# astooke/accel_rl

Hardware: AMD Instinct MI355X
Metric: env-steps/sec (whole node), 256-env PPO Atari (higher is better)
Workload: dtype f32; 1 GPU; PPO breakout, 256 envs/GPU, horizon 5, spec-1 CNN (fp32), minibatch 512/GPU x 4 epochs, adam; synthetic fixed-frame emulator; hipGraph rollout; total_envs=256, global_minibatch=512, parallelism=single

## Files before the change

accel_rl_amd/_lib.py:

```python
import ctypes as C
import os

import torch

_PKG = os.path.dirname(os.path.abspath(__file__))
LIB_PATH = os.path.join(_PKG, "libaccel_rl_hip.so")

ARL_ABI_VERSION = 4
PROMO_NEP50, PROMO_LEGACY, PROMO_ASSOC = 0, 1, 2
PPO_TIE_THEANO, PPO_TIE_MATH, PPO_TIE_BOTH = 0, 1, 2
OPT_ADAM, OPT_RMSPROP = 0, 1
MAX_ACTIONS = 18
REPLAY_MAX_HORIZON = 16
RAW_H, RAW_W, OBS_H, OBS_W = 210, 160, 104, 80
OPT_PARTIALS = 1024

_vp, _i32, _i64, _f32, _f64 = C.c_void_p, C.c_int32, C.c_int64, C.c_float, C.c_double


class ArlGame(C.Structure):
    _fields_ = [("bank", _vp), ("n_frames", _i32), ("n_actions", _i32),
                ("action_set", _i32 * MAX_ACTIONS), ("start_lives", _i32),
                ("life_period", _i32), ("frame_skip", _i32), ("n_stack", _i32),
                ("clip_reward", _i32), ("episodic_lives", _i32), ("resample_mode", _i32)]
# ... 157 lines not shown
    "arl_is_weights": (_i32, [_vp, _i64, _f64, _vp, _vp]),
    "arl_priority_diffs": (_i32, [_vp, _vp, _i64, _f64, _vp, _vp]),
    "arl_catdqn_act": (_i32, [_vp, _vp, _vp, _i64, _i32, _i32, _i32, _i32, _vp, _vp, _vp]),
    "arl_catdqn_loss": (_i32, [_vp] * 8 + [_i64, _i32, _i32, _i32, _i32, _f32, _f32, _f32, _vp, _vp, _vp, _vp]),
    "arl_catdqn_loss_parts": (_i32, [_vp] * 8 + [_i64, _i32, _i32, _i32, _i32, _f32, _f32, _f32, _vp, _vp, _vp, _vp, _i32,
                               _vp]),
    "arl_dqn_act": (_i32, [_vp, _vp, _i64, _i32, _i32, _i32, _vp, _vp, _vp]),
    "arl_dqn_loss": (_i32, [_vp] * 7 + [_i64, _i32, _i32, _i32, _f32, _f32, _vp, _vp, _vp, _vp]),
    "arl_lstm_cell_fwd": (_i32, [_vp, _i64, _vp, _vp, _i64, _i64, _i32, _vp, _i64, _vp, _i64, _vp, _i64, _vp]),
    "arl_lstm_cell_bwd": (_i32, [_vp, _i64, _vp, _vp, _vp, _i64, _vp, _i64, _vp, _i64, _i64, _i32, _vp, _i64, _vp, _vp]),
    "arl_gru_cell_fwd": (_i32, [_vp, _i64, _vp, _vp, _i64, _i64, _i32, _vp, _i64, _vp, _i64, _vp]),
    "arl_gru_cell_bwd": (_i32, [_vp, _i64, _vp, _vp, _vp, _i64, _vp, _i64, _i64, _i32, _vp, _i64, _vp, _i64, _vp, _vp]),
    "arl_rnn_cell_fwd": (_i32, [_vp, _i64, _vp, _i64, _i32, _vp, _i64, _vp]),
    "arl_rnn_cell_bwd": (_i32, [_vp, _i64, _vp, _vp, _i64, _i64, _i32, _vp, _i64, _vp]),
    "arl_opt_step": (_i32, [C.POINTER(ArlOptState), _i32, _f32, _f32, _f32, _f32, _f32, _f32, _vp]),
    "arl_opt_step_noclip": (_i32, [C.POINTER(ArlOptState), _i32, _f32, _f32, _f32, _f32, _f32, _i32, _vp, _vp, _vp]),
    "arl_opt_finish": (_i32, [C.POINTER(ArlOptState), _i32, _f32, _vp, _vp, _vp]),
    "arl_opt_step_noclip_split": (_i32, [C.POINTER(ArlOptState), _i32, _f32, _f32, _f32, _f32, _f32, _i32, _vp, _vp,
                                         _i64, _i64, _i32, _vp]),
    "arl_opt_finish_split": (_i32, [C.POINTER(ArlOptState), _i32, _f32, _vp, _vp, _i64, _vp]),
    "arl_corun_job_init": (_i32, [C.POINTER(ArlCorunJob), C.POINTER(ArlOptState), _i32, _f32, _f32, _f32, _f32, _f32,
                                  _i32, _vp, _vp, _i64, _i64]),
    "arl_corun_job_run": (_i32, [C.POINTER(ArlCorunJob), _vp]),
    "arl_noisy_normals": (_i32, [_i64, _i64, _i32, _i32, _i64, _i32, _i32, _vp, _vp, _vp, _vp]),
    "arl_noisy_noise": (_i32, [_vp, C.POINTER(ArlNoisyLayer), _i32, _i64, _i32, _vp]),
    "arl_noisy_dense_combine": (_i32, [C.POINTER(ArlFoldItem), _vp, C.POINTER(ArlFoldItem), _vp, _vp, _i64, _i32, _i32,
                                       _vp, _vp, _vp, _vp, _vp]),
    "arl_noisy_dense_bwd_prep": (_i32, [_vp, _vp, _i64, _i32, _vp, _vp, _vp, _vp]),
    "arl_noisy_dense_bwd_dx": (_i32, [_vp, _vp, _vp, _i64, _i32, _vp, _vp]),
    "arl_noisy_draws": (_i32, [_vp, C.POINTER(ArlNoisyDraw), _i32, _i64, _i32, _vp]),
    "arl_noisy_duel_combine": (_i32, [C.POINTER(ArlFoldItem), _vp, C.POINTER(ArlFoldItem), C.POINTER(ArlFoldItem), _vp,
                                      _vp, _i64, _i32, _i32, _i32, _vp, _vp, _vp, _vp, _vp]),
    "arl_noisy_duel_bwd_prep": (_i32, [_vp, _vp, _i64, _i32, _i32, _vp, _vp, _vp, _vp, _vp]),
    "arl_noisy_duel_bwd_dx": (_i32, [_vp, _vp, _vp, _vp, _vp, _i64, _i32, _vp, _vp]),
    "arl_noisy_catdqn_loss_limits": (_i32, [C.POINTER(_i32), C.POINTER(_i32), C.POINTER(_i32)]),
    "arl_noisy_catdqn_loss_parts": (_i32, [C.POINTER(ArlNoisyLogitSrc), C.POINTER(ArlNoisyLogitSrc),
                                           C.POINTER(ArlNoisyLogitSrc), _vp, _vp, _vp, _vp, _vp, _i64, _i32, _i32, _i32,
                                           _i32, _f32, _f32, _f32, _vp, _vp, _vp, C.POINTER(ArlDgradWt), _i32, _vp]),
}

_DEV_SIGNATURES = {
    "arl_dev_conv_trace_buffer": (None, [_vp]),
    "arl_dev_conv_force_generic": (None, [_i32]),
    "arl_dev_conv_variant": (None, [_i32]),
    "arl_dev_fwd_tile": (None, [_i32]),
    "arl_dev_dgrad_wt": (None, [_i32]),
# ... 507 lines not shown
    def pg_head_loss(self, h, w_head, b_head, actions, advantages, returns, old_prob, valids, idx, lr_mult,
                     inv_count, n_actions, kind, clip_param, v_loss_coeff, ent_loss_coeff,
                     dout, dh, dw_head, db_head, loss4, workspace, stream=None, relu_mask_dh=False,
                 tie_rule=PPO_TIE_THEANO, dgrad_weights=None):
        batch, hid = h.shape
        assert self._n + 3 <= FOLD_MAX_ITEMS, "too many pending folds"
        first = C.byref(self._items[self._n])
        self._n += 3
        wt_items, n_wt = None, 0
        if dgrad_weights:
            n_wt = len(dgrad_weights)
            assert n_wt <= DGRAD_WT_MAX
            wt_items = (ArlDgradWt * n_wt)()
            for it, (w, wt, geom) in zip(wt_items, dgrad_weights):
                it.w, it.wt, it.geom = ptr(w), ptr(wt), C.pointer(geom)
        _check(load().arl_pg_head_loss_parts(
            ptr(h), w_head.data_ptr(), b_head.data_ptr(), ptr(actions), ptr(advantages), ptr(returns),
            ptr(old_prob), ptr(valids), ptr(idx), ptr(lr_mult), ptr(inv_count), batch, hid, n_actions,
            kind, int(tie_rule), float(clip_param), float(v_loss_coeff), float(ent_loss_coeff), int(bool(relu_mask_dh)), ptr(dout),
            ptr(dh), dw_head.data_ptr(), db_head.data_ptr(), ptr(loss4), ptr(workspace), first,
            None if wt_items is None else C.cast(wt_items, _vp), n_wt, stream_ptr(stream)),
            "arl_pg_head_loss_parts")

    def run(self, stream=None):
        n, self._n = self._n, 0
        _check(load().arl_fold_many(self._items, n, stream_ptr(stream)), "arl_fold_many")



def replay_append(rb, observations, actions, rewards, dones, horizon, idx, discount, promo=PROMO_NEP50,
                  stream=None):
    _want(observations, torch.uint8, "observations")
    _want(actions, torch.uint8, "actions")
    _want(rewards, torch.float32, "rewards")
    _check(load().arl_replay_append(C.byref(rb), ptr(observations), ptr(actions), ptr(rewards), ptr(dones),
                                    horizon, idx, float(discount), promo, stream_ptr(stream)), "arl_replay_append")


def replay_extract(rb, env_idxs, step_idxs, obs, next_obs, actions, returns, terminals, stream=None):
    _want(env_idxs, torch.int32, "env_idxs")
    _want(step_idxs, torch.int32, "step_idxs")
    _check(load().arl_replay_extract(C.byref(rb), ptr(env_idxs), ptr(step_idxs), env_idxs.numel(), ptr(obs),
                                     ptr(next_obs), ptr(actions), ptr(returns), ptr(terminals),
                                     stream_ptr(stream)), "arl_replay_extract")


def sumtree_find(tree, levels, uniforms, out, stream=None):
    _want(tree, torch.float64, "tree")
    _want(uniforms, torch.float64, "uniforms")
# ... 297 lines not shown
```

accel_rl_amd/csrc/arl_optim_dev.h:

```cpp
#pragma once

#include "arl_common.h"

namespace arl {

__device__ __forceinline__ double wave_sum_d(double x) {
#pragma unroll
    for (int off = 32; off > 0; off >>= 1) x += __shfl_down(x, off, 64);
    return x;
}

__device__ __forceinline__ double block_sum_d(double x, double* lds) {
    x = wave_sum_d(x);
    const int lane = threadIdx.x & 63, w = threadIdx.x >> 6, nw = blockDim.x >> 6;
    if (lane == 0) lds[w] = x;
    __syncthreads();
    if (threadIdx.x == 0) {
        double s = 0;
        for (int i = 0; i < nw; ++i) s += lds[i];
        lds[0] = s;
    }
    __syncthreads();
    const double r = lds[0];
    __syncthreads();
// ... 70 lines not shown
        if (METHOD == ARL_OPT_ADAM) st_nt(v4 + i, v);
    }
    const long long n = o.n_params;
    if (c.finish && block == 0 && threadIdx.x < (n & 3)) {
        const long long i = ((n >> 2) << 2) + threadIdx.x;
        const float g = o.grads[i];
        float p = o.params[i], m = o.slot0[i], v = (METHOD == ARL_OPT_ADAM) ? o.slot1[i] : 0.f;
        s += (double)g * g;
        update_one<METHOD>(p, g, m, v, c.avg, 1.f, lr, a_t, c.b1, c.b2, c.eps);
        o.params[i] = p;
        o.slot0[i] = m;
        if (METHOD == ARL_OPT_ADAM) o.slot1[i] = v;
    }
    s = block_sum_d(s, lds);
    if (threadIdx.x == 0) {
        c.norm_parts[(long long)c.k * ARL_OPT_NORM_BLOCKS + c.block0 + block] = s;
        if (c.finish && block == 0) { c.step_pp[(c.k + 1) & 1] = t; o.step_count[0] = t; }
    }
    if (block == 0)
        for (int i = nblocks + threadIdx.x; i < c.slots; i += blockDim.x)
            c.norm_parts[(long long)c.k * ARL_OPT_NORM_BLOCKS + c.block0 + i] = 0.0;
}

inline void opt_split_plan(long long n_params, long long hole_count, int* rest, int* hole) {
    const long long n4 = n_params >> 2, h4 = hole_count >> 2;
    *rest = (int)stream_grid(n4 - h4, 256);
    if (h4 > 0 && *rest > ARL_OPT_NORM_BLOCKS / 2) *rest = ARL_OPT_NORM_BLOCKS / 2;
    long long hb = (h4 + 511) / 512;
    if (hb > ARL_OPT_NORM_BLOCKS - *rest) hb = ARL_OPT_NORM_BLOCKS - *rest;
    *hole = h4 > 0 ? (int)(hb < 1 ? 1 : hb) : 0;
}

int make_opt_seg(OptSeg* c, const arl_opt_state* opt, int32_t method, float learning_rate, float avg_factor,
                 float beta1_or_rho, float beta2, float epsilon, int32_t k, float* step_pp, double* norm_parts,
                 int64_t hole_first, int64_t hole_count, int part, int* blocks);
int launch_opt_seg(const OptSeg& c, int blocks, hipStream_t s);

}
```

accel_rl_amd/csrc/mfma_conv.hip:

```cpp
#include "mfma_conv_impl.h"
#include "dgrad_wt_dev.h"

using namespace arlc;

namespace arlc {
thread_local CallCtx t_ctx = {9, nullptr, false};
unsigned long long* g_trace = nullptr;
bool g_force_generic = false;
int g_fwd_tile = -1;
}

namespace {
constexpr int FOLD_WIDE = 128, FOLD_THREADS = 1024;
int g_fold_wide = FOLD_WIDE;
bool g_dgrad_wt = true;

struct FoldSlot { int64_t i; int zg, zgn, row0, o; };
__device__ __forceinline__ FoldSlot fold_slot(int splits, int local_block, int wide_from) {
    FoldSlot f;
    const int tid = threadIdx.x;
    f.o = tid & 15;
    if (splits >= wide_from) { f.zg = tid >> 4; f.zgn = 64; f.row0 = 0; f.i = (int64_t)local_block * 16 + f.o; }
    else {
        const int grp = tid >> 8;
// ... 55 lines not shown
};

__global__ __launch_bounds__(FOLD_THREADS) void fold_many_kernel(const FoldManyArgs a) {
    __shared__ float4 lds[64][16];
    int it = 0;
    while (it + 1 < a.n && (int)blockIdx.x >= a.block_start[it + 1]) ++it;
    const float4* part = reinterpret_cast<const float4*>(a.items[it].part);
    float4* out = reinterpret_cast<float4*>(a.items[it].out);
    const int64_t total4 = a.items[it].total >> 2;
    const int splits = a.items[it].splits;
    const FoldSlot f = fold_slot(splits, (int)blockIdx.x - a.block_start[it], a.wide_from);
    const float4 s = fold_sum(part, splits, total4, f, lds);
    const int64_t i = f.i;
    if (f.zg == 0 && i < total4) {
        const int64_t valid = a.items[it].valid;
        if (valid <= 0 || 4 * i + 3 < valid) {
            out[i] = s;
        } else {
            float* o1 = reinterpret_cast<float*>(out + i);
            if (4 * i < valid) o1[0] = s.x;
            if (4 * i + 1 < valid) o1[1] = s.y;
            if (4 * i + 2 < valid) o1[2] = s.z;
        }
    }
}

int launch_fold(const float* part, int splits, int64_t total, const float* bias, int n_bias, int relu,
                float* out, hipStream_t s, const float* mask = nullptr) {
    const int64_t total4 = total >> 2;
    hipLaunchKernelGGL(fold_splits_kernel, dim3((unsigned)fold_blocks(splits, total4)), dim3(FOLD_THREADS), 0, s,
                       (const float4*)part, splits, total4, (const float4*)bias, n_bias >> 2, relu,
                       (const float4*)mask, (float4*)out, g_fold_wide);
    return arl::check_launch("fold_splits_kernel");
}

}

extern "C" int64_t arl_conv_workspace_bytes(void) { return (int64_t)64 << 20; }

extern "C" void arl_dev_conv_trace_buffer(void* device_u64_or_null) { g_trace = (unsigned long long*)device_u64_or_null; }

extern "C" void arl_dev_conv_force_generic(int32_t on) { g_force_generic = on != 0; }

extern "C" void arl_dev_fold_wide_from(int32_t splits) { g_fold_wide = splits > 0 ? splits : FOLD_WIDE; }

extern "C" void arl_dev_fwd_tile(int32_t v) { g_fwd_tile = ((v >= 0 && v <= 2) || v == 6 || v == 7) ? v : -1; }
// ... 557 lines not shown
        for (int ph = 0; ph < st; ++ph)
            for (int pw = 0; pw < st; ++pw) {
                q.i0[ph * st + pw] = (ph + g.pad_h) % st;
                q.j0[ph * st + pw] = (pw + g.pad_w) % st;
            }
        a.block_start[i] = blocks;
        blocks += (q.total + 255) / 256;
    }
    a.block_start[n] = blocks; a.n = n;
    *blocks_out = blocks;
    return 0;
}
}

extern "C" int arl_conv2d_dgrad_weights(const arl_dgrad_wt* items, int32_t n, void* stream) {
    arlw::DgradWtArgs a;
    int blocks = 0;
    int rc = arlw::dgrad_wt_plan(items, n, &a, &blocks);
    if (rc) return rc;
    hipLaunchKernelGGL(dgrad_weights_kernel, dim3((unsigned)blocks), dim3(256), 0, (hipStream_t)stream, a);
    return arl::check_launch("dgrad_weights_kernel");
}

extern "C" int arl_fold_many(const arl_fold_item* items, int32_t n, void* stream) {
    ARL_REQUIRE(items || n == 0, ARL_E_ARG, "null pointer");
    ARL_REQUIRE(n >= 0 && n <= ARL_FOLD_MAX_ITEMS, ARL_E_RANGE, "too many fold items");
    FoldManyArgs a = {};
    int blocks = 0;
    for (int i = 0; i < n; ++i) {
        if (items[i].splits <= 0) continue;
        ARL_REQUIRE(items[i].part && items[i].out && items[i].total > 0 && (items[i].total & 3) == 0, ARL_E_ARG,
                    "fold item: null pointer or length not a multiple of 4");
        ARL_REQUIRE(arl::aligned16(items[i].part) && arl::aligned16(items[i].out), ARL_E_ALIGN, "16-byte alignment");
        a.items[a.n] = items[i];
        a.block_start[a.n++] = blocks;
        blocks += fold_blocks(items[i].splits, items[i].total >> 2);
    }
    if (a.n == 0) return 0;
    a.block_start[a.n] = blocks;
    a.wide_from = g_fold_wide;
    hipLaunchKernelGGL(fold_many_kernel, dim3((unsigned)blocks), dim3(FOLD_THREADS), 0, (hipStream_t)stream, a);
    return arl::check_launch("fold_many_kernel");
}
```

accel_rl_amd/optimizers/base.py:

```python
import numpy as np
import torch

from accel_rl_amd import _lib

NORM_LOG_LEN = 64


def iterate_mb_idxs(batch_size, data_length, shuffle=False):
    if shuffle:
        order = np.arange(data_length)
        np.random.shuffle(order)
    for lo in range(0, data_length - batch_size + 1, batch_size):
        yield order[lo:lo + batch_size] if shuffle else np.arange(lo, lo + batch_size)


def iterate_traj_idxs(batch_size, data_length, horizon=1, shuffle=False):
    if data_length % horizon or batch_size % horizon or data_length % batch_size:
        raise AssertionError("batch_size and data_length must be multiples of horizon, data_length of batch_size")
    rows = np.arange(data_length).reshape(-1, horizon)
    order = np.arange(data_length // horizon)
    per = batch_size // horizon
    if shuffle:
        np.random.shuffle(order)
    for lo in range(0, len(order), per):
# ... 11 lines not shown

    @property
    def parallelism_tag(self):
        raise NotImplementedError

    def _setup_bucket(self, target, lr_mult, givens=None):
        self._target = target
        dev = target.device
        n = target.flat_params.numel()
        self._slot0 = torch.zeros(n, dtype=torch.float32, device=dev)
        self._slot1 = torch.zeros(n, dtype=torch.float32, device=dev) \
            if self._update_method.name == "adam" else None
        self._step_count = torch.zeros(1, dtype=torch.float32, device=dev)
        if not isinstance(lr_mult, torch.Tensor):
            lr_mult = torch.full((1,), float(lr_mult), dtype=torch.float32, device=dev)
        self._lr_mult = lr_mult
        self._partials = torch.zeros(_lib.OPT_PARTIALS, dtype=torch.float64, device=dev)
        self._norm_log = torch.zeros(NORM_LOG_LEN, dtype=torch.float32, device=dev)
        self._n_updates = 0
        self._step_pp = self._norm_parts = None
        self._hole = None
        self._call_hole = None
        self._hole_count = 0
        st = _lib.ArlOptState()
        st.n_params = n
        st.params, st.grads = target.flat_params.data_ptr(), target.flat_grads.data_ptr()
        st.slot0 = self._slot0.data_ptr()
        st.slot1 = self._slot1.data_ptr() if self._slot1 is not None else None
        st.step_count, st.lr_mult = self._step_count.data_ptr(), self._lr_mult.data_ptr()
        st.partials, st.grad_norm_log = self._partials.data_ptr(), self._norm_log.data_ptr()
        st.norm_log_len = NORM_LOG_LEN
        self._opt_state = st
        a = self._update_args
        if self._update_method.name == "adam":
            self._kernel_args = (a["beta1"], a["beta2"], a["epsilon"])
        else:
            self._kernel_args = (a["rho"], 0.0, a["epsilon"])

    def _backward(self, losses, minibatch):
        return losses(minibatch)[3]

    def _apply_update(self, avg_factor=1.0):
        b1, b2, eps = self._kernel_args
        if self._grad_norm_clip is None:
            self._noclip_state()
            k = self._n_updates % self._opt_state.norm_log_len
            hole, self._hole = self._hole, None
            if k == 0:
                self._call_hole = hole
                self._hole_count = hole[1] if hole else 0
            elif self._hole_count and hole is None:
                hole = self._call_hole
                _lib.corun_job_run(_lib.corun_job(self._opt_state, self._update_method.kernel_id, self._learning_rate,
                                                  avg_factor, b1, b2, eps, k, self._step_pp, self._norm_parts,
                                                  hole[0], hole[1]))
            if self._hole_count:
                hole = self._call_hole
                _lib.opt_step_noclip_split(self._opt_state, self._update_method.kernel_id, self._learning_rate,
                                           avg_factor, b1, b2, eps, k, self._step_pp, self._norm_parts, hole[0],
                                           hole[1], 0)
            else:
                _lib.opt_step_noclip(self._opt_state, self._update_method.kernel_id, self._learning_rate, avg_factor,
                                     b1, b2, eps, k, self._step_pp, self._norm_parts)
            self._pending_avg = avg_factor
        else:
            _lib.opt_step(self._opt_state, self._update_method.kernel_id, self._learning_rate,
                          avg_factor, self._grad_norm_clip, b1, b2, eps)
        self._n_updates += 1

    corun_update = True

    def _noclip_state(self):
        if self._step_pp is None:
            dev = self._target.device
            self._step_pp = self._step_count.repeat(2).contiguous()
            self._norm_parts = torch.zeros(_lib.OPT_NORM_SLOTS * _lib.OPT_NORM_BLOCKS, dtype=torch.float64, device=dev)
        elif self._n_updates % self._opt_state.norm_log_len == 0 and not self._hole:
            self._step_pp.copy_(self._step_count.expand(2))

    def _corun_hook(self, avg_factor=1.0):
        if self._grad_norm_clip is not None or not self.corun_update:
            return None
        b1, b2, eps = self._kernel_args

        def hook(first, count):
            self._noclip_state()
            k = self._n_updates % self._opt_state.norm_log_len
            if k and (self._hole_count == 0 or self._call_hole != (first, count)):
                return None
            self._hole = (first, count)
            return _lib.corun_job(self._opt_state, self._update_method.kernel_id, self._learning_rate, avg_factor,
                                  b1, b2, eps, k, self._step_pp, self._norm_parts, first, count)
        return hook

    def _set_updates_per_call(self, count):
        count = max(1, min(int(count), NORM_LOG_LEN))
        if self._opt_state.norm_log_len != count:
            assert self._n_updates % count == 0 or self._n_updates == 0
            self._opt_state.norm_log_len = count

    def _recent_grad_norms(self, count):
        assert 0 < count <= self._opt_state.norm_log_len
        self._finish_updates(count)
        out = self._norm_log[:count]
        return out if (out.is_cuda and torch.cuda.is_current_stream_capturing()) else out.clone()

    def _finish_updates(self, count):
        if self._grad_norm_clip is None and self._step_pp is not None:
            _lib.opt_finish(self._opt_state, count, self._pending_avg, self._step_pp, self._norm_parts,
                            hole_count=self._hole_count)
```

accel_rl_amd/optimizers/single.py:

```python
import numpy as np
import torch

from accel_rl_amd import _lib

from accel_rl_amd.optimizers.base import BaseOptimizer, iterate_mb_idxs


class A2cOptimizer(BaseOptimizer):

    def __init__(self, learning_rate, update_method, update_method_args=None, grad_norm_clip=None):
        self._learning_rate = learning_rate
        self._update_method = update_method
        self._update_args = update_method.resolve(**(update_method_args or dict()))
        self._grad_norm_clip = grad_norm_clip

    def initialize(self, inputs, losses, constraints, target, givens=None, lr_mult=1):
        self._input_names = list(inputs)
        self._losses = losses
        self._setup_bucket(target, lr_mult, givens)

    def optimize(self, inputs):
        self.prepare_host(len(inputs[0]))
        return self.device_updates(inputs)

# ... 43 lines not shown

    def prepare_host(self, data_length):
        bs = self._minibatch_size
        flat = [mb for _ in range(self._epochs)
                for mb in iterate_mb_idxs(bs, data_length, self._shuffle)]
        if self._idx_host is None:
            shape = (max(len(flat), 1), bs)
            self._idx_host = torch.zeros(shape, dtype=torch.int32).pin_memory()
            self._idx_dev = torch.zeros(shape, dtype=torch.int32, device=self._target.device)
        self._n_minibatches = len(flat)
        self._set_updates_per_call(len(flat))
        if flat:
            self._idx_host.copy_(torch.from_numpy(np.stack(flat).astype(np.int32)))

    def device_updates(self, inputs):
        data = dict(zip(self._input_names, inputs))
        if not self._n_minibatches:
            return [], []
        _lib.copy_bytes(self._idx_dev, self._idx_host)
        if self._overlap_allreduce:
            return self._overlapped_minibatches(data)
        losses = []
        corun = self._corun_hook() if self.parallelism_tag == "single" else None
        try:
            for k in range(self._n_minibatches):
                mb = self._minibatch(data, self._idx_dev[k])
                if corun is not None:
                    mb["dense_w_hook"] = corun
                losses.append(self._backward(self._losses, mb))
                self._share_grad()
                self._apply_update(self._avg_factor())
        finally:
            self._hole = None
        return losses, self._recent_grad_norms(self._n_minibatches)

    def _minibatch(self, data, idx):
        return dict(data, idx=idx)

    _overlap_allreduce = False

    def _overlapped_minibatches(self, data):
        losses = []
        for k in range(self._n_minibatches):
            pending = []
            mb = self._minibatch(data, self._idx_dev[k])
            mb["split_hook"] = lambda: pending.append(self._share_grad_async(tail=True))
            losses.append(self._backward(self._losses, mb))
            pending.append(self._share_grad_async(tail=False) if pending else self._share_grad_async(None))
            self._wait_all(pending)
            self._apply_update(self._avg_factor())
        return losses, self._recent_grad_norms(self._n_minibatches)

    @staticmethod
    def _wait_all(pending):
        for work in pending:
            if work is not None:
# ... 15 lines not shown
```

accel_rl_amd/policies/atari_cnn_policy.py:

```python
import ctypes as C
import os

import numpy as np
import torch

from accel_rl_amd import _lib
from accel_rl_amd.distributions import Categorical
from accel_rl_amd.spaces import Discrete
from accel_rl_amd.util.seed import layer_rng

KIND_A2C, KIND_PPO = 0, 1


def _glorot_uniform(shape):
    receptive = int(np.prod(shape[2:]))
    fan_in, fan_out = shape[1] * receptive, shape[0] * receptive
    a = np.sqrt(6. / (fan_in + fan_out))
    return layer_rng().uniform(low=-a, high=a, size=shape).astype(np.float32)


def _norm_c(shape, std):
    out = np.random.randn(*shape).astype(np.float32)
    out *= std / np.sqrt(np.square(out).sum(axis=0, keepdims=True))
    return out
# ... 309 lines not shown
                       inv_count=None, tie_rule=_lib.PPO_TIE_THEANO):
        with torch.no_grad():
            idx = mb.get("idx")
            rows = mb["observations"].shape[0] if idx is None else idx.shape[0]
            limit = self.rows_per_pass()
            if limit and rows >= 3 * limit:
                return self._loss_and_grads_in_passes(mb, rows, limit, kind, clip_param, v_loss_coeff, ent_loss_coeff,
                                                      lr_mult, inv_count, tie_rule)
            x = self._scaled(mb["observations"], idx)
            b = x.shape[0]
            acts, hids = self._trunk(x)
            g, k_head = self.grads, self._k_head
            hid = self._hid_geom[-1][0]
            dout = self._buffer(("dout", b), (b, self.n_act + 1))
            dh = self._buffer(("dh", b), (b, hid))
            loss4 = self._buffer(("loss", b), (4,))
            wts = self._dgrad_weight_items(b) if os.environ.get("ARL_WT_IN_HEAD", "1") != "0" else []
            self._folds.pg_head_loss(hids[-1], self.params[k_head], self.params[k_head + 1], mb["actions"],
                              mb["advantages"], mb["returns"], mb.get("old_prob"), mb.get("valids"),
                              idx, lr_mult, inv_count, self.n_act, kind, clip_param, v_loss_coeff,
                              ent_loss_coeff, dout, dh, g[k_head], g[k_head + 1], loss4, self._loss_ws,
                              relu_mask_dh=True, tie_rule=tie_rule, dgrad_weights=wts)
            self._wt_fresh = bool(wts)
            try:
                self._backward_trunk(x, acts, hids, dh, masked=True, split_hook=mb.get("split_hook"),
                                     dense_w_hook=mb.get("dense_w_hook"))
            finally:
                self._wt_fresh = False
            return loss4

    max_rows_per_pass = None
    CACHE_BYTES = 256 << 20

    def rows_per_pass(self):
        if not isinstance(self.max_rows_per_pass, str):
            return self.max_rows_per_pass
        per_row = int(np.prod(self._obs_shape)) + 8 * sum(nf * ho * wo for nf, ci, sz, st, pad, ho, wo in self._conv_geom)
        return max(256, (self.CACHE_BYTES // per_row + 128) // 256 * 256)

    def _loss_and_grads_in_passes(self, mb, rows, limit, kind, clip_param, v_loss_coeff, ent_loss_coeff, lr_mult,
                                  inv_count, tie_rule=_lib.PPO_TIE_THEANO):
        idx = mb.get("idx")
        if idx is None:
            idx = self._buffer(("all_rows", rows), (rows,), dtype=torch.int32)
            idx.copy_(torch.arange(rows, dtype=torch.int32, device=self.device))
        if inv_count is None:
            inv_count = self._buffer(("inv_rows", rows), (1,))
            inv_count.fill_(1.0 / rows)
        if not getattr(self, "_passes_logged", False):
            self._passes_logged = True
            from accel_rl_amd.util import logger
            logger.log("AtariCnnPolicy: minibatches of %d rows are walked in passes of %d (gradients accumulated in a fixed "
                       "order; max_rows_per_pass = None keeps one pass)" % (rows, limit))
        acc = self._buffer(("grad_acc",), tuple(self.flat_grads.shape))
        loss_acc = self._buffer(("loss_acc",), (4,))
        one = dict((k, v) for k, v in mb.items() if k not in ("split_hook", "dense_w_hook"))
        saved, self.max_rows_per_pass = self.max_rows_per_pass, None
        try:
            for k, lo in enumerate(range(0, rows, limit)):
                one["idx"] = idx[lo:min(lo + limit, rows)]
                loss4 = self.loss_and_grads(one, kind, clip_param, v_loss_coeff, ent_loss_coeff, lr_mult, inv_count,
                                            tie_rule)
                if k == 0:
                    acc.copy_(self.flat_grads)
                    loss_acc.copy_(loss4)
                else:
                    acc.add_(self.flat_grads)
                    loss_acc.add_(loss4)
        finally:
            self.max_rows_per_pass = saved
        self.flat_grads.copy_(acc)
        hook = mb.get("split_hook")
        if hook is not None:
            hook()
        return loss_acc

    def _backward_trunk(self, x, acts, hids, dh, masked=False, split_hook=None, dense_w_hook=None):
        b = x.shape[0]
        conv_g, dense_g = self._layer_geoms(b)
# ... 16 lines not shown
        if not self._wt or _lib.default_route == _lib.ROUTE_FP32:
            return []
        conv_g, _ = self._layer_geoms(b)
        return [(self._w[2 * i], wt, conv_g[i]) for i, wt in sorted(self._wt.items())]

    def _backward_convs(self, x, acts, d_act, masked=False, corun=None):
        b = x.shape[0]
        conv_g, _ = self._layer_geoms(b)
        if not getattr(self, "_wt_fresh", False):
            items = self._dgrad_weight_items(b)
            if items:
                _lib.conv2d_dgrad_weights(items)
        for i in range(self._n_conv - 1, -1, -1):
            nf, ci, sz, st, pad, ho, wo = self._conv_geom[i]
            d_in = self._buffer(("dx_conv", i, b), tuple(acts[i - 1].shape)) if i > 0 else None
            self._layer_grads(d_act, masked, acts[i], b * ho * wo, nf, 2 * i, conv_g[i], acts[i - 1] if i > 0 else x, d_in,
                              corun=corun if i > 0 else None,
                              wt=self._wt.get(i) if _lib.default_route != _lib.ROUTE_FP32 else None)
            if corun is not None and i > 0 and self._folds.corun_taken:
                corun = None
            d_act, masked = d_in, True
        if corun is not None:
            _lib.corun_job_run(corun)
        self._folds.run()

    def _layer_grads(self, d, masked, y, rows, channels, k, geom, inp, d_in, corun=None, wt=None):
        folds, g = self._folds, self.grads
        if not masked:
            folds.relu_bwd_bias_grad(d, y, rows, channels, g[k + 1], self._fold_ws(("db", k)))
        dbias = g[k + 1] if masked else None
        if isinstance(inp, ObsRows):
            done = folds.conv2d_u8_bwd_weight(d, inp.obs, inp.idx, self._scale, self._g[k], geom,
                                              self._fold_ws(("dw", k)), dbias=dbias)
        elif d_in is not None:
            done = folds.conv2d_bwd_pair(d, self._w[k], inp, d_in, inp, self._g[k], geom, self._fold_ws(("dw", k)),
                                         dbias=dbias, corun=corun, wt=wt)
        else:
            done = folds.conv2d_bwd_weight(d, inp, self._g[k], geom, self._fold_ws(("dw", k)), dbias=dbias)
        if not done:
            folds.relu_bwd_bias_grad(d, y, rows, channels, g[k + 1], self._fold_ws(("db", k)))

    def _fold_ws(self, key):
        ws = self._fold_workspaces.get(key)
        if ws is None:
            ws = self._fold_workspaces[key] = (_lib.relu_bwd_workspace(self.device) if key[0] == "db"
                                               else _lib.conv_workspace(self.device))
        return ws
# ... 88 lines not shown
```

include/accel_rl_hip.h:

```cpp
#ifndef ACCEL_RL_HIP_H
#define ACCEL_RL_HIP_H

#include <stdint.h>

#ifdef __cplusplus
extern "C" {
#endif

#define ARL_ABI_VERSION 4

#define ARL_E_ARG      (-1)
#define ARL_E_RANGE    (-2)
#define ARL_E_ALIGN    (-3)

#define ARL_PROMO_NEP50   0
#define ARL_PROMO_LEGACY  1
#define ARL_PROMO_ASSOC   2

int         arl_abi_version(void);
const char* arl_last_error(void);


int arl_gae_scan(const float* rewards, const float* values, const uint8_t* dones,
                 const float* last_values, double discount, double gae_lambda,
// ... 376 lines not shown
} arl_opt_state;

#define ARL_OPT_PARTIALS 1024
#define ARL_OPT_ADAM     0
#define ARL_OPT_RMSPROP  1

int arl_opt_step(const arl_opt_state* opt, int32_t method, float learning_rate,
                 float avg_factor, float clip, float beta1_or_rho, float beta2,
                 float epsilon, void* stream);

#define ARL_OPT_NORM_SLOTS  64
#define ARL_OPT_NORM_BLOCKS 2048
int arl_opt_step_noclip(const arl_opt_state* opt, int32_t method, float learning_rate, float avg_factor,
                        float beta1_or_rho, float beta2, float epsilon, int32_t k, float* step_pp,
                        double* norm_parts, void* stream);
int arl_opt_finish(const arl_opt_state* opt, int32_t n_updates, float avg_factor, float* step_pp,
                   const double* norm_parts, void* stream);

int arl_opt_step_noclip_split(const arl_opt_state* opt, int32_t method, float learning_rate, float avg_factor,
                              float beta1_or_rho, float beta2, float epsilon, int32_t k, float* step_pp,
                              double* norm_parts, int64_t hole_first, int64_t hole_count, int32_t part, void* stream);
int arl_opt_finish_split(const arl_opt_state* opt, int32_t n_updates, float avg_factor, float* step_pp,
                         const double* norm_parts, int64_t hole_count, void* stream);
typedef struct arl_corun_job { int64_t opaque[40]; } arl_corun_job;
int arl_corun_job_init(arl_corun_job* job, const arl_opt_state* opt, int32_t method, float learning_rate,
                       float avg_factor, float beta1_or_rho, float beta2, float epsilon, int32_t k, float* step_pp,
                       double* norm_parts, int64_t hole_first, int64_t hole_count);
int arl_corun_job_run(const arl_corun_job* job, void* stream);


int arl_noisy_normals(int64_t seed, int64_t counter, int32_t layer, int32_t which, int64_t rows, int32_t width,
                      int32_t rows_per_draw, float* e_or_null, float* f_or_null, uint32_t* words_or_null,
                      void* stream);

typedef struct arl_noisy_layer {
    float* fein;
    float* feout;
    const float* x;
    float* xs;
    int32_t fan_in;
    int32_t units;
    int32_t out_stride;
    int32_t layer;
} arl_noisy_layer;
#define ARL_NOISY_MAX_LAYERS 8

// ... 67 lines not shown
```

Before: 366,200 env-steps/s.

## Fuse gradient fold reduction with Adam update and norm partials

Adds a kernel that reduces the split-K gradient partials for each fold item and immediately applies the optimizer update to those parameters. The same kernel updates the parameter ranges not covered by folds and computes per-chunk grad-norm partials, using atomic tickets to detect when a chunk is complete. This removes the separate optimizer-step launch and a re-read of grads, params and moment buffers after the fold. In exchange the planning logic is complex, it falls back to the plain fold when ranges overlap oddly, and it depends on correct cross-block atomic ordering.

```diff
diff --git a/accel_rl_amd/_lib.py b/accel_rl_amd/_lib.py
--- a/accel_rl_amd/_lib.py
+++ b/accel_rl_amd/_lib.py
@@ -203,6 +203,8 @@
     "arl_corun_job_init": (_i32, [C.POINTER(ArlCorunJob), C.POINTER(ArlOptState), _i32, _f32, _f32, _f32, _f32, _f32,
                                   _i32, _vp, _vp, _i64, _i64]),
     "arl_corun_job_run": (_i32, [C.POINTER(ArlCorunJob), _vp]),
+    "arl_fold_many_update": (_i32, [C.POINTER(ArlFoldItem), _i32, C.POINTER(ArlOptState), _i32, _f32, _f32, _f32, _f32,
+                                    _f32, _i32, _vp, _vp, _i64, _i64, _vp, C.POINTER(_i32), _vp]),
     "arl_noisy_normals": (_i32, [_i64, _i64, _i32, _i32, _i64, _i32, _i32, _vp, _vp, _vp, _vp]),
     "arl_noisy_noise": (_i32, [_vp, C.POINTER(ArlNoisyLayer), _i32, _i64, _i32, _vp]),
     "arl_noisy_dense_combine": (_i32, [C.POINTER(ArlFoldItem), _vp, C.POINTER(ArlFoldItem), _vp, _vp, _i64, _i32, _i32,
@@ -756,9 +758,24 @@
             None if wt_items is None else C.cast(wt_items, _vp), n_wt, stream_ptr(stream)),
             "arl_pg_head_loss_parts")
 
-    def run(self, stream=None):
+    def run(self, stream=None, update=None):
         n, self._n = self._n, 0
+        if update is not None:
+            update(self._items, n, stream)
+            return
         _check(load().arl_fold_many(self._items, n, stream_ptr(stream)), "arl_fold_many")
+
+
+def fold_many_update(items, n, opt, method, learning_rate, avg_factor, beta1_or_rho, beta2, epsilon, k, step_pp,
+                     norm_parts, hole_first, hole_count, tickets, stream=None):
+    _want(tickets, torch.int32, "tickets")
+    if tickets.numel() < OPT_NORM_BLOCKS:
+        raise ValueError("fold_many_update: tickets must hold OPT_NORM_BLOCKS words")
+    hosted = _i32(0)
+    _check(load().arl_fold_many_update(items, n, C.byref(opt), method, learning_rate, avg_factor, beta1_or_rho, beta2,
+                                       epsilon, int(k), ptr(step_pp), ptr(norm_parts), int(hole_first), int(hole_count),
+                                       ptr(tickets), C.byref(hosted), stream_ptr(stream)), "arl_fold_many_update")
+    return bool(hosted.value)
 
 
 
diff --git a/accel_rl_amd/csrc/arl_optim_dev.h b/accel_rl_amd/csrc/arl_optim_dev.h
--- a/accel_rl_amd/csrc/arl_optim_dev.h
+++ b/accel_rl_amd/csrc/arl_optim_dev.h
@@ -116,6 +116,15 @@
             c.norm_parts[(long long)c.k * ARL_OPT_NORM_BLOCKS + c.block0 + i] = 0.0;
 }
 
+template <int METHOD>
+__device__ __forceinline__ void opt_scalars(const OptSeg& c, float& t, float& lr, float& a_t) {
+    t = c.step_pp[c.k & 1] + 1.0f;
+    lr = c.lr_base * c.o.lr_mult[0];
+    a_t = 0.f;
+    if (METHOD == ARL_OPT_ADAM)
+        a_t = lr * sqrtf(1.f - powf(c.b2, t)) / (1.f - powf(c.b1, t));
+}
+
 inline void opt_split_plan(long long n_params, long long hole_count, int* rest, int* hole) {
     const long long n4 = n_params >> 2, h4 = hole_count >> 2;
     *rest = (int)stream_grid(n4 - h4, 256);
diff --git a/accel_rl_amd/csrc/mfma_conv.hip b/accel_rl_amd/csrc/mfma_conv.hip
--- a/accel_rl_amd/csrc/mfma_conv.hip
+++ b/accel_rl_amd/csrc/mfma_conv.hip
@@ -101,6 +101,197 @@
             if (4 * i + 1 < valid) o1[1] = s.y;
             if (4 * i + 2 < valid) o1[2] = s.z;
         }
+    }
+}
+
+constexpr int FOLD_MAX_GAPS = ARL_FOLD_MAX_ITEMS + 4;
+struct FoldUpdArgs {
+    FoldManyArgs f;
+    arl::OptSeg seg;
+    long long js0[ARL_FOLD_MAX_ITEMS];
+    long long gap_e[FOLD_MAX_GAPS];
+    long long gap_js[FOLD_MAX_GAPS];
+    int gap_len[FOLD_MAX_GAPS];
+    int gap_block[FOLD_MAX_GAPS + 1];
+    int n_gaps, tail;
+    long long seg_floats;
+    unsigned* tickets;
+};
+
+template <int METHOD>
+__device__ __forceinline__ void fold_upd_one(const arl::OptSeg& c, long long e, float g, float lr, float a_t) {
+    const arl_opt_state& o = c.o;
+    float p = o.params[e], m = o.slot0[e], v = (METHOD == ARL_OPT_ADAM) ? o.slot1[e] : 0.f;
+    arl::update_one<METHOD>(p, g, m, v, c.avg, 1.f, lr, a_t, c.b1, c.b2, c.eps);
+    o.params[e] = p;
+    o.slot0[e] = m;
+    if (METHOD == ARL_OPT_ADAM) o.slot1[e] = v;
+}
+
+__device__ __forceinline__ void store_wt(float* q, float x) {
+    typedef __attribute__((address_space(1))) unsigned gu32;
+    __hip_atomic_store((gu32*)q, __float_as_uint(x), __ATOMIC_RELAXED, __HIP_MEMORY_SCOPE_AGENT);
+}
+
+template <int METHOD>
+__global__ __launch_bounds__(FOLD_THREADS) void fold_many_update_kernel(const FoldUpdArgs a) {
+    __shared__ float4 lds[64][16];
+    __shared__ double lds_d[4];
+    __shared__ int lds_mask;
+    const arl::OptSeg& c = a.seg;
+    const int tid = threadIdx.x;
+    const int gap_first = a.f.block_start[a.f.n];
+    long long js_lo = 0, js_hi = 0;
+    bool tail_piece = false;
+    if ((int)blockIdx.x < gap_first) {
+        int it = 0;
+        while (it + 1 < a.f.n && (int)blockIdx.x >= a.f.block_start[it + 1]) ++it;
+        const arl_fold_item& item = a.f.items[it];
+        const float4* part = reinterpret_cast<const float4*>(item.part);
+        float4* out = reinterpret_cast<float4*>(item.out);
+        const int64_t total4 = item.total >> 2;
+        const int splits = item.splits;
+        const int local = (int)blockIdx.x - a.f.block_start[it];
+        const FoldSlot f = fold_slot(splits, local, a.f.wide_from);
+        const int64_t i = f.i;
+        const int64_t valid = item.valid;
+        const long long len = valid > 0 ? valid : item.total;
+        const bool hosted = a.js0[it] >= 0;
+        const bool mine = f.zg == 0 && i < total4;
+        const long long e = (item.out - c.o.grads) + 4 * i;
+        const bool four = hosted && mine && 4 * i + 3 < len;
+        float4 p = make_float4(0, 0, 0, 0), m = p, v = p;
+        float t = 0.f, lr = 0.f, a_t = 0.f;
+        if (hosted && mine) arl::opt_scalars<METHOD>(c, t, lr, a_t);
+        if (four) {
+            p = *reinterpret_cast<const float4*>(c.o.params + e);
+            m = *reinterpret_cast<const float4*>(c.o.slot0 + e);
+            if (METHOD == ARL_OPT_ADAM) v = *reinterpret_cast<const float4*>(c.o.slot1 + e);
+        }
+        const float4 s = fold_sum(part, splits, total4, f, lds);
+        if (mine) {
+            if (hosted) {
+                if (4 * i < len) store_wt(reinterpret_cast<float*>(out + i), s.x);
+                if (4 * i + 1 < len) store_wt(reinterpret_cast<float*>(out + i) + 1, s.y);
+                if (4 * i + 2 < len) store_wt(reinterpret_cast<float*>(out + i) + 2, s.z);
+                if (4 * i + 3 < len) store_wt(reinterpret_cast<float*>(out + i) + 3, s.w);
+            } else if (valid <= 0 || 4 * i + 3 < valid) {
+                out[i] = s;
+            } else {
+                float* o1 = reinterpret_cast<float*>(out + i);
+                if (4 * i < valid) o1[0] = s.x;
+                if (4 * i + 1 < valid) o1[1] = s.y;
+                if (4 * i + 2 < valid) o1[2] = s.z;
+            }
+            if (hosted && 4 * i < len) {
+                if (four) {
+                    arl::update_one<METHOD>(p.x, s.x, m.x, v.x, c.avg, 1.f, lr, a_t, c.b1, c.b2, c.eps);
+                    arl::update_one<METHOD>(p.y, s.y, m.y, v.y, c.avg, 1.f, lr, a_t, c.b1, c.b2, c.eps);
+                    arl::update_one<METHOD>(p.z, s.z, m.z, v.z, c.avg, 1.f, lr, a_t, c.b1, c.b2, c.eps);
+                    arl::update_one<METHOD>(p.w, s.w, m.w, v.w, c.avg, 1.f, lr, a_t, c.b1, c.b2, c.eps);
+                    *reinterpret_cast<float4*>(c.o.params + e) = p;
+                    *reinterpret_cast<float4*>(c.o.slot0 + e) = m;
+                    if (METHOD == ARL_OPT_ADAM) *reinterpret_cast<float4*>(c.o.slot1 + e) = v;
+                } else {
+                    fold_upd_one<METHOD>(c, e, s.x, lr, a_t);
+                    if (4 * i + 1 < len) fold_upd_one<METHOD>(c, e + 1, s.y, lr, a_t);
+                    if (4 * i + 2 < len) fold_upd_one<METHOD>(c, e + 2, s.z, lr, a_t);
+                }
+            }
+        }
+        if (a.js0[it] >= 0) {
+            const long long per = (splits >= a.f.wide_from ? 16 : 64) * 4;
+            const long long lo = (long long)local * per;
+            const long long hi = lo + per < len ? lo + per : len;
+            if (lo < hi) { js_lo = a.js0[it] + lo; js_hi = a.js0[it] + hi; }
+        }
+    } else {
+        const int g = (int)blockIdx.x - gap_first;
+        int r = 0;
+        while (r + 1 < a.n_gaps && g >= a.gap_block[r + 1]) ++r;
+        float t, lr, a_t;
+        arl::opt_scalars<METHOD>(c, t, lr, a_t);
+        if (a.gap_js[r] < 0) {
+            tail_piece = true;
+            if (tid < a.gap_len[r]) {
+                const long long e = a.gap_e[r] + tid;
+                fold_upd_one<METHOD>(c, e, c.o.grads[e], lr, a_t);
+            }
+        } else {
+            const long long g_lo = a.gap_js[r], g_hi = g_lo + a.gap_len[r];
+            const long long chunk = (g_lo >> 10) + (g - a.gap_block[r]);
+            js_lo = g_lo > (chunk << 10) ? g_lo : (chunk << 10);
+            js_hi = g_hi < ((chunk + 1) << 10) ? g_hi : ((chunk + 1) << 10);
+            const long long js = js_lo + tid;
+            if (js < js_hi) {
+                const long long e = a.gap_e[r] + (js - g_lo);
+                fold_upd_one<METHOD>(c, e, c.o.grads[e], lr, a_t);
+            }
+        }
+    }
+    if (blockIdx.x == 0 && tid == 0) {
+        const float t = c.step_pp[c.k & 1] + 1.0f;
+        c.step_pp[(c.k + 1) & 1] = t;
+        c.o.step_count[0] = t;
+    }
+    int n_ch = 0;
+    long long ch[2] = {0, 0};
+    unsigned cnt[2] = {0, 0};
+    if (tail_piece) { n_ch = 1; ch[0] = 0; cnt[0] = (unsigned)a.tail; }
+    else if (js_lo < js_hi) {
+        const long long c0 = js_lo >> 10, c1 = (js_hi - 1) >> 10;
+        const long long end0 = js_hi < ((c0 + 1) << 10) ? js_hi : ((c0 + 1) << 10);
+        n_ch = 1; ch[0] = c0; cnt[0] = (unsigned)(end0 - js_lo);
+        if (c1 != c0) { n_ch = 2; ch[1] = c1; cnt[1] = (unsigned)(js_hi - (c1 << 10)); }
+    }
+    asm volatile("s_waitcnt vmcnt(0)" ::: "memory");
+    __syncthreads();
+    if (tid == 0) {
+        int mask = 0;
+        if (n_ch) {
+            for (int q = 0; q < n_ch; ++q) {
+                long long want = a.seg_floats - (ch[q] << 10);
+                if (want > 1024) want = 1024;
+                if (ch[q] == 0) want += a.tail;
+                const unsigned old = __hip_atomic_fetch_add(a.tickets + ch[q], cnt[q], __ATOMIC_RELAXED,
+                                                            __HIP_MEMORY_SCOPE_AGENT);
+                if ((long long)old + cnt[q] == want) mask |= 1 << q;
+            }
+            if (mask) {
+                __builtin_amdgcn_fence(__ATOMIC_ACQUIRE, "agent");
+                asm volatile("s_waitcnt vmcnt(0)" ::: "memory");
+            }
+        }
+        lds_mask = mask;
+    }
+    __syncthreads();
+    const int mask = lds_mask;
+    for (int q = 0; q < 2; ++q) {
+        if (!((mask >> q) & 1)) continue;
+        const long long chunk = ch[q];
+        double s = 0;
+        if (tid < 256) {
+            const long long j = chunk * 256 + tid;
+            if (j < c.an + c.bn) {
+                const long long i4 = j < c.an ? c.a0 + j : c.b0 + (j - c.an);
+                const float4 g = reinterpret_cast<const float4*>(c.o.grads)[i4];
+                s += (double)g.x * g.x + (double)g.y * g.y + (double)g.z * g.z + (double)g.w * g.w;
+            }
+            if (chunk == 0 && tid < a.tail) {
+                const float g = c.o.grads[((c.o.n_params >> 2) << 2) + tid];
+                s += (double)g * g;
+            }
+            s = arl::wave_sum_d(s);
+            if ((tid & 63) == 0) lds_d[tid >> 6] = s;
+        }
+        __syncthreads();
+        if (tid == 0) {
+            double r = 0;
+            for (int w = 0; w < 4; ++w) r += lds_d[w];
+            c.norm_parts[(long long)c.k * ARL_OPT_NORM_BLOCKS + c.block0 + chunk] = r;
+            __hip_atomic_store(a.tickets + chunk, 0u, __ATOMIC_RELAXED, __HIP_MEMORY_SCOPE_AGENT);
+        }
+        __syncthreads();
     }
 }
 
@@ -704,23 +895,128 @@
     return arl::check_launch("dgrad_weights_kernel");
 }
 
-extern "C" int arl_fold_many(const arl_fold_item* items, int32_t n, void* stream) {
+namespace {
+int fold_plan(const arl_fold_item* items, int32_t n, FoldManyArgs* a, int* blocks_out) {
     ARL_REQUIRE(items || n == 0, ARL_E_ARG, "null pointer");
     ARL_REQUIRE(n >= 0 && n <= ARL_FOLD_MAX_ITEMS, ARL_E_RANGE, "too many fold items");
-    FoldManyArgs a = {};
+    *a = FoldManyArgs{};
     int blocks = 0;
     for (int i = 0; i < n; ++i) {
         if (items[i].splits <= 0) continue;
         ARL_REQUIRE(items[i].part && items[i].out && items[i].total > 0 && (items[i].total & 3) == 0, ARL_E_ARG,
                     "fold item: null pointer or length not a multiple of 4");
         ARL_REQUIRE(arl::aligned16(items[i].part) && arl::aligned16(items[i].out), ARL_E_ALIGN, "16-byte alignment");
-        a.items[a.n] = items[i];
-        a.block_start[a.n++] = blocks;
+        a->items[a->n] = items[i];
+        a->block_start[a->n++] = blocks;
         blocks += fold_blocks(items[i].splits, items[i].total >> 2);
     }
+    a->block_start[a->n] = blocks;
+    a->wide_from = g_fold_wide;
+    *blocks_out = blocks;
+    return 0;
+}
+
+int launch_fold_many(const FoldManyArgs& a, int blocks, hipStream_t s) {
     if (a.n == 0) return 0;
-    a.block_start[a.n] = blocks;
-    a.wide_from = g_fold_wide;
-    hipLaunchKernelGGL(fold_many_kernel, dim3((unsigned)blocks), dim3(FOLD_THREADS), 0, (hipStream_t)stream, a);
+    hipLaunchKernelGGL(fold_many_kernel, dim3((unsigned)blocks), dim3(FOLD_THREADS), 0, s, a);
     return arl::check_launch("fold_many_kernel");
 }
+
+bool fold_update_plan(FoldUpdArgs* u, int rest_blocks, int* gap_blocks) {
+    const arl::OptSeg& c = u->seg;
+    const long long n = c.o.n_params, total4 = c.an + c.bn;
+    if (total4 <= 0 || (long long)rest_blocks != (total4 + 255) / 256) return false;
+    u->seg_floats = 4 * total4;
+    u->tail = (int)(n & 3);
+    const long long a_lo = 4 * c.a0, a_hi = 4 * (c.a0 + c.an), b_lo = 4 * c.b0, b_hi = 4 * (c.b0 + c.bn);
+    struct Iv { long long lo, hi; };
+    Iv iv[ARL_FOLD_MAX_ITEMS];
+    int n_iv = 0;
+    const uintptr_t g0 = reinterpret_cast<uintptr_t>(c.o.grads), g1 = g0 + 4 * (uintptr_t)n;
+    for (int q = 0; q < u->f.n; ++q) {
+        const arl_fold_item& it = u->f.items[q];
+        const long long len = it.valid > 0 ? it.valid : it.total;
+        const uintptr_t o0 = reinterpret_cast<uintptr_t>(it.out), o1 = o0 + 4 * (uintptr_t)len;
+        u->js0[q] = -1;
+        if (o1 <= g0 || o0 >= g1) continue;
+        if (o0 < g0 || o1 > g1) return false;
+        const long long lo = (long long)((o0 - g0) >> 2), hi = lo + len;
+        if (c.an > 0 && lo >= a_lo && hi <= a_hi) u->js0[q] = lo - a_lo;
+        else if (c.bn > 0 && lo >= b_lo && hi <= b_hi) u->js0[q] = 4 * c.an + (lo - b_lo);
+        else if (lo >= a_hi && hi <= b_lo) continue;
+        else return false;
+        iv[n_iv++] = Iv{lo, hi};
+    }
+    for (int i = 1; i < n_iv; ++i)
+        for (int j = i; j > 0 && iv[j].lo < iv[j - 1].lo; --j) { const Iv t = iv[j]; iv[j] = iv[j - 1]; iv[j - 1] = t; }
+    for (int i = 1; i < n_iv; ++i)
+        if (iv[i].lo < iv[i - 1].hi) return false;
+    int ng = 0, gb = 0;
+    auto add_gap = [&](long long e_lo, long long e_hi, long long js) {
+        while (e_lo < e_hi) {
+            if (ng >= FOLD_MAX_GAPS) return false;
+            const long long len = e_hi - e_lo < (1LL << 30) ? e_hi - e_lo : (1LL << 30);
+            u->gap_e[ng] = e_lo; u->gap_js[ng] = js; u->gap_len[ng] = (int)len; u->gap_block[ng] = gb;
+            gb += (int)(((js + len - 1) >> 10) - (js >> 10) + 1);
+            ++ng; e_lo += len; js += len;
+        }
+        return true;
+    };
+    const Iv ranges[2] = {{a_lo, a_hi}, {b_lo, b_hi}};
+    const long long js_of[2] = {0, 4 * c.an};
+    for (int r = 0; r < 2; ++r) {
+        long long pos = ranges[r].lo;
+        for (int i = 0; i < n_iv && pos < ranges[r].hi; ++i) {
+            if (iv[i].hi <= ranges[r].lo || iv[i].lo >= ranges[r].hi) continue;
+            if (iv[i].lo > pos && !add_gap(pos, iv[i].lo, js_of[r] + (pos - ranges[r].lo))) return false;
+            pos = iv[i].hi;
+        }
+        if (pos < ranges[r].hi && !add_gap(pos, ranges[r].hi, js_of[r] + (pos - ranges[r].lo))) return false;
+    }
+    if (u->tail) {
+        if (ng >= FOLD_MAX_GAPS) return false;
+        u->gap_e[ng] = (n >> 2) << 2; u->gap_js[ng] = -1; u->gap_len[ng] = u->tail; u->gap_block[ng] = gb;
+        gb += 1; ++ng;
+    }
+    u->gap_block[ng] = gb;
+    u->n_gaps = ng;
+    *gap_blocks = gb;
+    return true;
+}
+}
+
+extern "C" int arl_fold_many(const arl_fold_item* items, int32_t n, void* stream) {
+    FoldManyArgs a;
+    int blocks = 0;
+    int rc = fold_plan(items, n, &a, &blocks);
+    if (rc) return rc;
+    return launch_fold_many(a, blocks, (hipStream_t)stream);
+}
+
+extern "C" int arl_fold_many_update(const arl_fold_item* items, int32_t n, const arl_opt_state* opt, int32_t method,
+                                    float learning_rate, float avg_factor, float beta1_or_rho, float beta2,
+                                    float epsilon, int32_t k, float* step_pp, double* norm_parts, int64_t hole_first,
+                                    int64_t hole_count, uint32_t* tickets, int32_t* hosted, void* stream) {
+    ARL_REQUIRE(hosted && tickets, ARL_E_ARG, "null pointer");
+    ARL_REQUIRE(arl::aligned4(tickets), ARL_E_ALIGN, "tickets: 4-byte alignment");
+    *hosted = 0;
+    FoldUpdArgs u = {};
+    int blocks = 0, rest = 0, gap_blocks = 0;
+    int rc = fold_plan(items, n, &u.f, &blocks);
+    if (rc) return rc;
+    rc = arl::make_opt_seg(&u.seg, opt, method, learning_rate, avg_factor, beta1_or_rho, beta2, epsilon, k, step_pp,
+                           norm_parts, hole_first, hole_count, 0, &rest);
+    if (rc) return rc;
+    u.tickets = tickets;
+    if (!fold_update_plan(&u, rest, &gap_blocks))
+        return launch_fold_many(u.f, blocks, (hipStream_t)stream);
+    const dim3 grid((unsigned)(blocks + gap_blocks));
+    if (method == ARL_OPT_ADAM)
+        hipLaunchKernelGGL((fold_many_update_kernel<ARL_OPT_ADAM>), grid, dim3(FOLD_THREADS), 0, (hipStream_t)stream, u);
+    else
+        hipLaunchKernelGGL((fold_many_update_kernel<ARL_OPT_RMSPROP>), grid, dim3(FOLD_THREADS), 0, (hipStream_t)stream, u);
+    rc = arl::check_launch("fold_many_update_kernel");
+    if (rc) return rc;
+    *hosted = 1;
+    return 0;
+}
diff --git a/accel_rl_amd/optimizers/base.py b/accel_rl_amd/optimizers/base.py
--- a/accel_rl_amd/optimizers/base.py
+++ b/accel_rl_amd/optimizers/base.py
@@ -1,3 +1,5 @@
+import os
+
 import numpy as np
 import torch
 
@@ -57,6 +59,8 @@
         self._hole = None
         self._call_hole = None
         self._hole_count = 0
+        self._update_hosted = None
+        self._tickets = None
         st = _lib.ArlOptState()
         st.n_params = n
         st.params, st.grads = target.flat_params.data_ptr(), target.flat_grads.data_ptr()
@@ -78,7 +82,8 @@
     def _apply_update(self, avg_factor=1.0):
         b1, b2, eps = self._kernel_args
         if self._grad_norm_clip is None:
-            self._noclip_state()
+            if self._update_hosted is None:
+                self._noclip_state()
             k = self._n_updates % self._opt_state.norm_log_len
             hole, self._hole = self._hole, None
             if k == 0:
@@ -89,7 +94,10 @@
                 _lib.corun_job_run(_lib.corun_job(self._opt_state, self._update_method.kernel_id, self._learning_rate,
                                                   avg_factor, b1, b2, eps, k, self._step_pp, self._norm_parts,
                                                   hole[0], hole[1]))
-            if self._hole_count:
+            hosted, self._update_hosted = self._update_hosted, None
+            if hosted is not None:
+                assert hosted == (k, self._call_hole, avg_factor), "the hosted update is not the one due now"
+            elif self._hole_count:
                 hole = self._call_hole
                 _lib.opt_step_noclip_split(self._opt_state, self._update_method.kernel_id, self._learning_rate,
                                            avg_factor, b1, b2, eps, k, self._step_pp, self._norm_parts, hole[0],
@@ -128,6 +136,26 @@
                                   b1, b2, eps, k, self._step_pp, self._norm_parts, first, count)
         return hook
 
+    fold_update = True
+
+    def _fold_update_hook(self, avg_factor=1.0):
+        if self._grad_norm_clip is not None or not self.fold_update or os.environ.get("ARL_FOLD_UPDATE", "1") == "0":
+            return None
+        b1, b2, eps = self._kernel_args
+
+        def hook(items, n, stream=None):
+            self._noclip_state()
+            if self._tickets is None:
+                self._tickets = torch.zeros(_lib.OPT_NORM_BLOCKS, dtype=torch.int32, device=self._target.device)
+            k = self._n_updates % self._opt_state.norm_log_len
+            hole = self._hole if k == 0 else (self._call_hole if self._hole_count else None)
+            first, count = hole if hole else (0, 0)
+            if _lib.fold_many_update(items, n, self._opt_state, self._update_method.kernel_id, self._learning_rate,
+                                     avg_factor, b1, b2, eps, k, self._step_pp, self._norm_parts, first, count,
+                                     self._tickets, stream):
+                self._update_hosted = (k, hole, avg_factor)
+        return hook
+
     def _set_updates_per_call(self, count):
         count = max(1, min(int(count), NORM_LOG_LEN))
         if self._opt_state.norm_log_len != count:
diff --git a/accel_rl_amd/optimizers/single.py b/accel_rl_amd/optimizers/single.py
--- a/accel_rl_amd/optimizers/single.py
+++ b/accel_rl_amd/optimizers/single.py
@@ -89,16 +89,20 @@
             return self._overlapped_minibatches(data)
         losses = []
         corun = self._corun_hook() if self.parallelism_tag == "single" else None
+        fold_update = self._fold_update_hook() if self.parallelism_tag == "single" else None
         try:
             for k in range(self._n_minibatches):
                 mb = self._minibatch(data, self._idx_dev[k])
                 if corun is not None:
                     mb["dense_w_hook"] = corun
+                if fold_update is not None:
+                    mb["fold_update_hook"] = fold_update
                 losses.append(self._backward(self._losses, mb))
                 self._share_grad()
                 self._apply_update(self._avg_factor())
         finally:
             self._hole = None
+            self._update_hosted = None
         return losses, self._recent_grad_norms(self._n_minibatches)
 
     def _minibatch(self, data, idx):
diff --git a/accel_rl_amd/policies/atari_cnn_policy.py b/accel_rl_amd/policies/atari_cnn_policy.py
--- a/accel_rl_amd/policies/atari_cnn_policy.py
+++ b/accel_rl_amd/policies/atari_cnn_policy.py
@@ -355,11 +355,13 @@
                               ent_loss_coeff, dout, dh, g[k_head], g[k_head + 1], loss4, self._loss_ws,
                               relu_mask_dh=True, tie_rule=tie_rule, dgrad_weights=wts)
             self._wt_fresh = bool(wts)
+            self._fold_update = mb.get("fold_update_hook")
             try:
                 self._backward_trunk(x, acts, hids, dh, masked=True, split_hook=mb.get("split_hook"),
                                      dense_w_hook=mb.get("dense_w_hook"))
             finally:
                 self._wt_fresh = False
+                self._fold_update = None
             return loss4
 
     max_rows_per_pass = None
@@ -387,7 +389,7 @@
                        "order; max_rows_per_pass = None keeps one pass)" % (rows, limit))
         acc = self._buffer(("grad_acc",), tuple(self.flat_grads.shape))
         loss_acc = self._buffer(("loss_acc",), (4,))
-        one = dict((k, v) for k, v in mb.items() if k not in ("split_hook", "dense_w_hook"))
+        one = dict((k, v) for k, v in mb.items() if k not in ("split_hook", "dense_w_hook", "fold_update_hook"))
         saved, self.max_rows_per_pass = self.max_rows_per_pass, None
         try:
             for k, lo in enumerate(range(0, rows, limit)):
@@ -450,7 +452,7 @@
             d_act, masked = d_in, True
         if corun is not None:
             _lib.corun_job_run(corun)
-        self._folds.run()
+        self._folds.run(update=getattr(self, "_fold_update", None))
 
     def _layer_grads(self, d, masked, y, rows, channels, k, geom, inp, d_in, corun=None, wt=None):
         folds, g = self._folds, self.grads
diff --git a/include/accel_rl_hip.h b/include/accel_rl_hip.h
--- a/include/accel_rl_hip.h
+++ b/include/accel_rl_hip.h
@@ -422,6 +422,10 @@
                               double* norm_parts, int64_t hole_first, int64_t hole_count, int32_t part, void* stream);
 int arl_opt_finish_split(const arl_opt_state* opt, int32_t n_updates, float avg_factor, float* step_pp,
                          const double* norm_parts, int64_t hole_count, void* stream);
+int arl_fold_many_update(const arl_fold_item* items, int32_t n, const arl_opt_state* opt, int32_t method,
+                         float learning_rate, float avg_factor, float beta1_or_rho, float beta2, float epsilon,
+                         int32_t k, float* step_pp, double* norm_parts, int64_t hole_first, int64_t hole_count,
+                         uint32_t* tickets, int32_t* hosted, void* stream);
 typedef struct arl_corun_job { int64_t opaque[40]; } arl_corun_job;
 int arl_corun_job_init(arl_corun_job* job, const arl_opt_state* opt, int32_t method, float learning_rate,
                        float avg_factor, float beta1_or_rho, float beta2, float epsilon, int32_t k, float* step_pp,
```

Result: no change. 366,100 env-steps/s (-0.0%).
